# Dorothy-2016/rgbd360

Hardware: AMD Instinct MI355X
Metric: registered Frame360 pairs/sec @ 8×640×480; ICP-reduce HBM GB/s vs roofline (higher is better)
Workload: dtype f32

## Files before the change

### rgbd360_amd/csrc/kernels/plane_seg.hip

```cpp
#include <cstdio>
#include <cstdlib>
#include <cstring>
#include <type_traits>
#include "../r360_internal.h"
#include "../plane_math.h"

namespace {

__device__ __forceinline__ bool isfin(float v) { return __builtin_isfinite(v); }

__device__ __forceinline__ int ld(const int* p) { return __hip_atomic_load(p, __ATOMIC_RELAXED, __HIP_MEMORY_SCOPE_AGENT); }

__device__ int find_root(int* parent, int x) {
    int p = ld(parent + x);
    while (p != x) {
        const int gp = ld(parent + p);
        if (gp != p) __hip_atomic_store(parent + x, gp, __ATOMIC_RELAXED, __HIP_MEMORY_SCOPE_AGENT);
        x = gp;
        p = ld(parent + x);
    }
    return x;
}

__device__ void unite(int* parent, int a, int b) {
    while (true) {
        a = find_root(parent, a);
        b = find_root(parent, b);
        if (a == b) return;
        if (a < b) { const int t = a; a = b; b = t; }
        const int old = atomicCAS(parent + a, a, b);
        if (old == a) return;
        a = old;
    }
}

__device__ __forceinline__ bool plane_cmp(const float4& pa, const float4& na, const float4& nb, float ang_thr) {
    float thr = 0.02f;
    const float z = pa.x * 0.f + pa.y * 0.f + pa.z * 1.f;
    thr *= z * z;
    const float nd = na.x * nb.x + na.y * nb.y + na.z * nb.z;
    return fabsf(na.w - nb.w) < thr && nd > ang_thr;
}

constexpr int CCL_ROWS = 16, CCL_TPB = 1024;

__device__ int lds_find(int* lp, int x) {
    int p = lp[x];
    while (p != x) {
        const int gp = lp[p];
        if (gp != p) lp[x] = gp;
        x = gp;
        p = lp[x];
    }
    return x;
}

__device__ void lds_unite(int* lp, int a, int b) {
    while (true) {
        a = lds_find(lp, a);
        b = lds_find(lp, b);
        if (a == b) return;
        if (a < b) { const int t = a; a = b; b = t; }
        const int old = atomicCAS(lp + a, a, b);
        if (old == a) return;
        a = old;
    }
}

__device__ __forceinline__ void d_ccl_local(const float4* __restrict__ cloud, const float4* __restrict__ nrm,
                                                      int w, int h, float ang_thr, int* __restrict__ parent) {
    extern __shared__ int lp[];
    const int s = blockIdx.y, r0 = blockIdx.x * CCL_ROWS;
    if (r0 >= h) return;
    const int rows = min(CCL_ROWS, h - r0), n = rows * w;
    const long base = (long)s * w * h + (long)r0 * w;
    for (int k = threadIdx.x; k < n; k += CCL_TPB) lp[k] = isfin(cloud[base + k].x) ? k : -1;
    __syncthreads();
    for (int k = threadIdx.x; k < n; k += CCL_TPB) {
        if (lp[k] < 0) continue;
        const int rr = k / w, c = k - rr * w;
        const float4 p = cloud[base + k], nn = nrm[base + k];
        if (c >= 1 && lp[k - 1] >= 0 && plane_cmp(p, nn, nrm[base + k - 1], ang_thr)) lds_unite(lp, k, k - 1);
        if (rr >= 1 && lp[k - w] >= 0 && plane_cmp(p, nn, nrm[base + k - w], ang_thr)) lds_unite(lp, k, k - w);
    }
    __syncthreads();
    for (int k = threadIdx.x; k < n; k += CCL_TPB) {
        const int v = lp[k];
        parent[base + k] = v < 0 ? -1 : (int)(base + lds_find(lp, k));
    }
}
__global__ void __launch_bounds__(CCL_TPB) k_ccl_local(const PlaneBatch B, int w, int h, float ang_thr) {
    const PlaneDev& D = B.f[blockIdx.z];
    d_ccl_local(D.cloud, D.nrm, w, h, ang_thr, D.parent);
}


__device__ __forceinline__ void d_ccl_border(const float4* __restrict__ cloud, const float4* __restrict__ nrm, int w, int h,
                             float ang_thr, int* __restrict__ parent) {
    const int nb = (h - 1) / CCL_ROWS;
    const long total = 8L * nb * w;
    for (long t = blockIdx.x * (long)blockDim.x + threadIdx.x; t < total; t += (long)gridDim.x * blockDim.x) {
        const int s = (int)(t / ((long)nb * w));
        const int q = (int)(t - (long)s * nb * w);
        const int b = q / w, c = q - b * w;
        const long i = (long)s * w * h + (long)(b + 1) * CCL_ROWS * w + c;
        if (ld(parent + i) < 0 || ld(parent + i - w) < 0) continue;
        if (plane_cmp(cloud[i], nrm[i], nrm[i - w], ang_thr)) unite(parent, (int)i, (int)(i - w));
    }
}
__global__ void k_ccl_border(const PlaneBatch B, int w, int h, float ang_thr) {
    const PlaneDev& D = B.f[blockIdx.z];
    d_ccl_border(D.cloud, D.nrm, w, h, ang_thr, D.parent);
}


constexpr int NUMC = 256;

__device__ __forceinline__ void d_ccl_flatten(int* __restrict__ parent, int N, int* __restrict__ root,
                                                     int* __restrict__ cnt, int* __restrict__ ccnt) {
    const int s = blockIdx.y, j = blockIdx.x * NUMC + threadIdx.x;
    const long i = (long)s * N + j;
    bool is_root = false;
    if (j < N) {
        const int r = parent[i] < 0 ? -1 : find_root(parent, (int)i);
        root[i] = r;
        cnt[i] = 0;
        is_root = r == (int)i;
    }
    const int c = __syncthreads_count(is_root);
    if (threadIdx.x == 0) ccnt[s * gridDim.x + blockIdx.x] = c;
}
__global__ void __launch_bounds__(NUMC) k_ccl_flatten(const PlaneBatch B, int N) {
    const PlaneDev& D = B.f[blockIdx.z];
    d_ccl_flatten(D.parent, N, D.root, D.cnt, D.chunk);
}


__device__ __forceinline__ int chunk_rank(bool flag, const int* __restrict__ ccnt_s, int chunk, int& off, int& tot) {
    __shared__ int s_w[NUMC / 64], s_off[NUMC / 64];
    const int lane = threadIdx.x & 63, wid = threadIdx.x >> 6;
    int a = 0;
    for (int k = threadIdx.x; k < chunk; k += NUMC) a += ccnt_s[k];
    for (int o = 32; o > 0; o >>= 1) a += __shfl_xor(a, o, 64);
    const unsigned long long m = __ballot(flag);
    if (lane == 0) { s_off[wid] = a; s_w[wid] = __popcll(m); }
    __syncthreads();
    int o = 0, before = 0, t = 0;
    for (int w = 0; w < NUMC / 64; ++w) { o += s_off[w]; before += w < wid ? s_w[w] : 0; t += s_w[w]; }
    off = o;
    tot = t;
    return before + (int)__builtin_amdgcn_mbcnt_hi((unsigned)(m >> 32), __builtin_amdgcn_mbcnt_lo((unsigned)m, 0u));
}

__device__ __forceinline__ void d_ccl_number(const int* __restrict__ root, int N, const int* __restrict__ ccnt,
                                                    int* __restrict__ rank, int* __restrict__ nlab) {
    const int s = blockIdx.y, j = blockIdx.x * NUMC + threadIdx.x;
    const long i = (long)s * N + j;
    const bool is_root = j < N && root[i] == (int)i;
    int off, tot;
    const int r = chunk_rank(is_root, ccnt + s * gridDim.x, blockIdx.x, off, tot);
    if (is_root) rank[i] = off + r;
    if (blockIdx.x == gridDim.x - 1 && threadIdx.x == 0) nlab[s] = off + tot;
}
__global__ void __launch_bounds__(NUMC) k_ccl_number(const PlaneBatch B, int N) {
    const PlaneDev& D = B.f[blockIdx.z];
    d_ccl_number(D.root, N, D.chunk, D.parent, D.nlab);
}


__device__ __forceinline__ void d_ccl_label(const int* __restrict__ root, const int* __restrict__ rank, int N, int* __restrict__ lab,
                            int* __restrict__ cnt) {
    const long total = 8L * N;
    for (long i = blockIdx.x * (long)blockDim.x + threadIdx.x; i < total; i += (long)gridDim.x * blockDim.x) {
        const int rt = root[i];
        const int L = rt < 0 ? -1 : rank[rt];
        lab[i] = L;
        const int s = (int)(i / N);
        long key = L < 0 ? -1 : (long)s * N + L;
        bool pending = key >= 0;
        while (__any(pending)) {
            const unsigned long long act = __ballot(pending);
            const int leader = __ffsll((long long)act) - 1;
            const long lk = __shfl(key, leader, 64);
            const bool mine = pending && key == lk;
            const unsigned long long same = __ballot(mine);
            if (mine && (int)(threadIdx.x & 63) == leader) atomicAdd(cnt + lk, __popcll(same));
            if (mine) pending = false;
        }
    }
}
__global__ void k_ccl_label(const PlaneBatch B, int N) {
    const PlaneDev& D = B.f[blockIdx.z];
    d_ccl_label(D.root, D.parent, N, D.lab, D.cnt);
}


__device__ __forceinline__ void atomic_fmin(float* p, float v) {
    if (v >= 0.f) atomicMin(reinterpret_cast<int*>(p), __float_as_int(v));
    else atomicMax(reinterpret_cast<unsigned*>(p), __float_as_uint(v));
}
__device__ __forceinline__ void atomic_fmax(float* p, float v) {
    if (v >= 0.f) atomicMax(reinterpret_cast<int*>(p), __float_as_int(v));
    else atomicMin(reinterpret_cast<unsigned*>(p), __float_as_uint(v));
}

__device__ __forceinline__ void add128(unsigned long long* p, r360p::i128 v) {
    const unsigned long long lo = (unsigned long long)v, hi = (unsigned long long)(v >> 64);
    const unsigned long long old = atomicAdd(p, lo);
    atomicAdd(p + 1, hi + (old + lo < old ? 1ull : 0ull));
}

__device__ __forceinline__ void d_big_count(const int* __restrict__ cnt, const int* __restrict__ nlab, int N,
                                                   int min_inliers, int* __restrict__ bmap, int* __restrict__ ccnt) {
    const int s = blockIdx.y, j = blockIdx.x * NUMC + threadIdx.x;
    const long i = (long)s * N + j;
    bool big = false;
    if (j < nlab[s]) {
        big = cnt[i] > min_inliers;
        if (!big) bmap[i] = -1;
    }
    const int c = __syncthreads_count(big);
    if (threadIdx.x == 0) ccnt[s * gridDim.x + blockIdx.x] = c;
}
__global__ void __launch_bounds__(NUMC) k_big_count(const PlaneBatch B, int N, int min_inliers) {
    const PlaneDev& D = B.f[blockIdx.z];
    d_big_count(D.cnt, D.nlab, N, min_inliers, D.parent, D.chunk);
}


__device__ __forceinline__ void d_big_list(const int* __restrict__ cnt, const int* __restrict__ nlab, int N,
                                                  int min_inliers, const int* __restrict__ ccnt, int* __restrict__ big,
                                                  int* __restrict__ nbig, int maxbig, int* __restrict__ err,
                                                  int* __restrict__ bmap, r360p::Moments* __restrict__ mom,
                                                  int* __restrict__ bfirst) {
    const int s = blockIdx.y, j = blockIdx.x * NUMC + threadIdx.x;
    const long i = (long)s * N + j;
    const bool is_big = j < nlab[s] && cnt[i] > min_inliers;
    int off, tot;
    const int r = chunk_rank(is_big, ccnt + s * gridDim.x, blockIdx.x, off, tot);
    if (is_big) {
        const int b = off + r;
        bmap[i] = b < maxbig ? b : -1;
        if (b < maxbig) big[s * maxbig + b] = j;
    }
    if (blockIdx.x == gridDim.x - 1) {
        const int all = off + tot, nb = all < maxbig ? all : maxbig;
        if (threadIdx.x == 0) {
            nbig[s] = nb;
            if (all > maxbig) atomicOr(err, 2);
        }
        for (int q = threadIdx.x; q < nb; q += NUMC) {
            r360p::moments_zero(mom[s * maxbig + q]);
            bfirst[s * maxbig + q] = N;
        }
    }
}
__global__ void __launch_bounds__(NUMC) k_big_list(const PlaneBatch B, int N, int min_inliers, int maxbig) {
    const PlaneDev& D = B.f[blockIdx.z];
    d_big_list(D.cnt, D.nlab, N, min_inliers, D.chunk, D.big, D.nbig, maxbig, D.err, D.parent, D.mom, D.aux);
}


constexpr int GM_TPB = 256, GM_SLOTS = 64, GM_PX = 512, GM_COPIES = R360_GM_COPIES;


struct GmShared {
    int key[GM_SLOTS];
    unsigned long long w[GM_SLOTS][20];
    float b[GM_SLOTS][6];
    int first[GM_SLOTS];
};

struct GmAcc {
    long long n, s1[3], c[4];
    r360p::i128 s2[6];
    float b[6];
    int first;
};

__device__ __forceinline__ void gm_zero(GmAcc& a) {
    a.n = 0;
    a.first = 0x7fffffff;
    for (int k = 0; k < 3; ++k) a.s1[k] = 0;
    for (int k = 0; k < 4; ++k) a.c[k] = 0;
    for (int k = 0; k < 6; ++k) { a.s2[k] = 0; a.b[k] = k < 3 ? 3.4e38f : -3.4e38f; }
}


template <bool MODEL>
__device__ __forceinline__ void gm_deposit(GmShared* sh, int key, const GmAcc& a, r360p::Moments* gmom, int* gfirst,
                                           RegionPart* gout) {
    int h = key & (GM_SLOTS - 1), t = 0;
#pragma unroll 1
    for (; t < GM_SLOTS; ++t, h = (h + 1) & (GM_SLOTS - 1)) {
        const int old = atomicCAS(&sh->key[h], -1, key);
        if (old == -1 || old == key) break;
    }
    if (t < GM_SLOTS) {
        unsigned long long* d = sh->w[h];
        if (a.n) {
            atomicAdd(d + 0, (unsigned long long)a.n);
            for (int k = 0; k < 3; ++k) atomicAdd(d + 1 + k, (unsigned long long)a.s1[k]);
            for (int k = 0; k < 6; ++k) add128(d + 4 + 2 * k, a.s2[k]);
        }
        if (MODEL) {
            for (int k = 0; k < 4; ++k) atomicAdd(d + 16 + k, (unsigned long long)a.c[k]);
            for (int k = 0; k < 3; ++k) { atomic_fmin(&sh->b[h][k], a.b[k]); atomic_fmax(&sh->b[h][k + 3], a.b[k + 3]); }
        } else {
            atomicMin(&sh->first[h], a.first);
        }
        return;
    }
    r360p::Moments* dst = MODEL ? &gout[key].m : &gmom[key];
    if (a.n) {
        atomicAdd(reinterpret_cast<unsigned long long*>(&dst->n), (unsigned long long)a.n);
        for (int k = 0; k < 3; ++k) atomicAdd(reinterpret_cast<unsigned long long*>(&dst->s1[k]), (unsigned long long)a.s1[k]);
        for (int k = 0; k < 6; ++k) add128(reinterpret_cast<unsigned long long*>(&dst->s2[k]), a.s2[k]);
    }
    if (MODEL) {
        for (int k = 0; k < 4; ++k) atomicAdd(reinterpret_cast<unsigned long long*>(&dst->c[k]), (unsigned long long)a.c[k]);
        for (int k = 0; k < 3; ++k) { atomic_fmin(&gout[key].bmin[k], a.b[k]); atomic_fmax(&gout[key].bmax[k], a.b[k + 3]); }
    } else {
        atomicMin(gfirst + key, a.first);
    }
}

template <int CTRL>
__device__ __forceinline__ unsigned dpp32(unsigned v) {
    return (unsigned)__builtin_amdgcn_update_dpp(0, (int)v, CTRL, 0xf, 0xf, false);
}
template <int CTRL>
__device__ __forceinline__ long long dpp64(long long v) {
    const unsigned lo = dpp32<CTRL>((unsigned)(unsigned long long)v), hi = dpp32<CTRL>((unsigned)((unsigned long long)v >> 32));
    return (long long)(((unsigned long long)hi << 32) | lo);
}
template <int CTRL>
__device__ __forceinline__ r360p::i128 dpp128(r360p::i128 v) {
    const unsigned long long lo = (unsigned long long)dpp64<CTRL>((long long)(unsigned long long)v);
    const unsigned long long hi = (unsigned long long)dpp64<CTRL>((long long)(unsigned long long)(v >> 64));
    return (r360p::i128)(((unsigned __int128)hi << 64) | lo);
}
template <bool MODEL, int CTRL>
__device__ __forceinline__ void gm_scan_step(GmAcc& v, bool take) {
    long long s1[3];
    r360p::i128 s2[6];
    for (int k = 0; k < 3; ++k) s1[k] = dpp64<CTRL>(v.s1[k]);
    for (int k = 0; k < 6; ++k) s2[k] = dpp128<CTRL>(v.s2[k]);
    if (MODEL) {
        long long c[4];
        float b[6];
        for (int k = 0; k < 4; ++k) c[k] = dpp64<CTRL>(v.c[k]);
        for (int k = 0; k < 6; ++k) b[k] = __uint_as_float(dpp32<CTRL>(__float_as_uint(v.b[k])));
        if (take) {
            for (int k = 0; k < 4; ++k) v.c[k] += c[k];
            for (int k = 0; k < 3; ++k) { v.b[k] = fminf(v.b[k], b[k]); v.b[k + 3] = fmaxf(v.b[k + 3], b[k + 3]); }
        }
    }
    if (take) {
        for (int k = 0; k < 3; ++k) v.s1[k] += s1[k];
        for (int k = 0; k < 6; ++k) v.s2[k] += s2[k];
    }
}
template <bool MODEL>
__device__ __forceinline__ void gm_seg_scan(GmAcc& v, int lane, int head) {
    const int r = lane & 15, row = lane >> 4;
    gm_scan_step<MODEL, 0x111>(v, r >= 1 && head <= lane - 1);
    gm_scan_step<MODEL, 0x112>(v, r >= 2 && head <= lane - 2);
    gm_scan_step<MODEL, 0x114>(v, r >= 4 && head <= lane - 4);
    gm_scan_step<MODEL, 0x118>(v, r >= 8 && head <= lane - 8);
    gm_scan_step<MODEL, 0x142>(v, (row & 1) && head <= (lane & ~15) - 1);
    gm_scan_step<MODEL, 0x143>(v, row >= 2 && head <= 31);
}

template <bool MODEL, int CPW>
__device__ __forceinline__ void d_gm(const float4* __restrict__ cloud, const uchar4* __restrict__ rgb,
                                             const int* __restrict__ lab, int N, const int* __restrict__ kmap,
                                             int* __restrict__ mmap_clear, const float* __restrict__ rt8,
                                             r360p::Moments* __restrict__ gmom, int* __restrict__ gfirst,
                                             RegionPart* __restrict__ gpart, int exp) {
    __shared__ GmShared sh;
    RegionPart* const gout = MODEL ? gpart + (blockIdx.x % GM_COPIES) * 8 * R360_MAX_MODELS : nullptr;
    for (int q = threadIdx.x; q < GM_SLOTS; q += GM_TPB) {
        sh.key[q] = -1;
        sh.first[q] = 0x7fffffff;
        for (int k = 0; k < 20; ++k) sh.w[q][k] = 0;
        for (int k = 0; k < 6; ++k) sh.b[q][k] = k < 3 ? 3.4e38f : -3.4e38f;
    }
    const int lane = threadIdx.x & 63, wid = threadIdx.x >> 6;
    const long total = 8L * N;
    const long w0 = ((long)blockIdx.x * GM_TPB * CPW) + (long)wid * 64 * CPW + lane;
    int key[CPW];
#pragma unroll
    for (int c = 0; c < CPW; ++c) {
        const long i = w0 + 64 * c;
        key[c] = i < total ? lab[i] : -1;
        if (!MODEL && i < total) mmap_clear[i] = -1;
    }
#pragma unroll
    for (int c = 0; c < CPW; ++c) {
        const long i = w0 + 64 * c;
        const int s = (int)(i / N);
        const int m = key[c] >= 0 ? kmap[(long)s * N + key[c]] : -1;
        key[c] = m >= 0 ? s * (MODEL ? R360_MAX_MODELS : R360_MAX_BIG) + m : -1;
    }
    float4 pt[CPW];
    uchar4 col[CPW];
#pragma unroll
    for (int c = 0; c < CPW; ++c) {
        const long i = w0 + 64 * c;
        pt[c] = key[c] >= 0 ? cloud[i] : make_float4(0.f, 0.f, 0.f, 0.f);
        if (MODEL) col[c] = key[c] >= 0 ? rgb[i] : make_uchar4(0, 0, 0, 0);
    }
    __syncthreads();
#pragma unroll
    for (int c = 0; c < CPW; ++c) {
        const long i = w0 + 64 * c;
        const int s = (int)(i / N);
        GmAcc p;
        gm_zero(p);
        if (key[c] >= 0) {
            const float4 q = pt[c];
            float x = q.x, y = q.y, z = q.z;
            bool add = true;
            if (MODEL) {
                p.b[0] = q.x; p.b[1] = q.y; p.b[2] = q.z; p.b[3] = q.x; p.b[4] = q.y; p.b[5] = q.z;
                const float* T = rt8 + 16 * s;
                x = T[0] * q.x + T[4] * q.y + T[8] * q.z + T[12];
                y = T[1] * q.x + T[5] * q.y + T[9] * q.z + T[13];
                z = T[2] * q.x + T[6] * q.y + T[10] * q.z + T[14];
                const uchar4 cc = col[c];
                const int sum = cc.x + cc.y + cc.z;
                if (sum != 0) {
                    const float inv = 1.0f / float(sum);
                    p.c[0] = (long long)((double)(float(cc.x) * inv) * 8589934592.0);
                    p.c[1] = (long long)((double)(float(cc.y) * inv) * 8589934592.0);
                    p.c[2] = (long long)((double)(float(cc.z) * inv) * 8589934592.0);
                }
                p.c[3] = sum;
            } else {
                p.first = (int)(i - (long)s * N);
                add = isfin(q.x) && isfin(q.y) && isfin(q.z);
            }
            if (add) {
                const long long qv[3] = {r360p::q36(x), r360p::q36(y), r360p::q36(z)};
                p.n = 1;
                for (int k = 0; k < 3; ++k) p.s1[k] = qv[k];
                p.s2[0] = (r360p::i128)qv[0] * qv[0];
                p.s2[1] = (r360p::i128)qv[0] * qv[1];
                p.s2[2] = (r360p::i128)qv[0] * qv[2];
                p.s2[3] = (r360p::i128)qv[1] * qv[1];
                p.s2[4] = (r360p::i128)qv[1] * qv[2];
                p.s2[5] = (r360p::i128)qv[2] * qv[2];
            }
        }
        const unsigned long long heads = __ballot(lane == 0 || key[c] != __shfl_up(key[c], 1, 64));
        const unsigned long long le = lane == 63 ? ~0ull : (2ull << lane) - 1;
        const int head = 63 - __clzll((long long)(heads & le));
        const unsigned long long fin = __ballot(p.n != 0);
        if (!(exp & 4)) gm_seg_scan<MODEL>(p, lane, head);
        const bool tail = lane == 63 || ((heads >> (lane + 1)) & 1ull);
        if (!(exp & 2) && tail && key[c] >= 0) {
            const unsigned long long run = le & ~((1ull << head) - 1);
            p.n = __popcll(fin & run);
            p.first -= lane - head;
            gm_deposit<MODEL>(&sh, key[c], p, gmom, gfirst, gout);
        }
    }
    __syncthreads();
    for (int q = threadIdx.x >> 5; q < GM_SLOTS; q += GM_TPB / 32) {
        const int key = sh.key[q];
        if (key < 0 || (exp & 1)) continue;
        const int l = threadIdx.x & 31;
        r360p::Moments* dst = MODEL ? &gout[key].m : &gmom[key];
        if (l < 6) {
            unsigned long long* d = reinterpret_cast<unsigned long long*>(&dst->s2[l]);
            const unsigned long long lo = sh.w[q][4 + 2 * l], hi = sh.w[q][5 + 2 * l];
            const unsigned long long old = atomicAdd(d, lo);
            atomicAdd(d + 1, hi + (old + lo < old ? 1ull : 0ull));
        } else if (l < 14) {
            const int k = l - 6;
            if (k < 4 || MODEL) {
                long long* d = k == 0 ? &dst->n : k < 4 ? &dst->s1[k - 1] : &dst->c[k - 4];
                atomicAdd(reinterpret_cast<unsigned long long*>(d), sh.w[q][k == 0 ? 0 : k < 4 ? k : 12 + k]);
            }
        } else if (MODEL && l < 20) {
            const int k = l - 14;
            if (k < 3) atomic_fmin(&gout[key].bmin[k], sh.b[q][k]);
            else atomic_fmax(&gout[key].bmax[k - 3], sh.b[q][k]);
        } else if (!MODEL && l == 14) {
            atomicMin(gfirst + key, sh.first[q]);
        }
    }
}
template <bool MODEL, int CPW>
// ... 1426 lines not shown
        totals[1] = pre + x;
        if (pre + x > vox_cap) atomicOr(err, 16);
    }
}
__global__ void __launch_bounds__(512) k_vox_alloc(const PlaneBatch B) {
    const PlaneDev& D = B.f[blockIdx.z];
    d_vox_alloc(D.nmodels, D.out, D.totals, D.vox_cap, D.err);
}


constexpr int VOXC_TPB = 256;

template <typename F>
__device__ __forceinline__ void wave_by_key(int key, F&& f) {
    bool pending = key >= 0;
    while (__any(pending)) {
        const unsigned long long act = __ballot(pending);
        const int leader = __ffsll((long long)act) - 1;
        const int lk = __shfl(key, leader, 64);
        const bool mine = pending && key == lk;
        f(lk, __ballot(mine), leader, mine);
        if (mine) pending = false;
    }
}

__device__ __forceinline__ void d_vox_compact(VoxCell* __restrict__ tab,
                                                         const long* __restrict__ totals, PlaneOut* __restrict__ out,
                                                         VoxOut* __restrict__ pool, long pool_cap,
                                                         const int* __restrict__ vlist, const int* __restrict__ vcnt,
                                                         int px) {
    if (totals[3] == 0) return;
    const int n = vcnt[blockIdx.x];
    if (n == 0) return;
    __shared__ int cnt[8 * R360_MAX_MODELS], base[8 * R360_MAX_MODELS];
    for (int q = threadIdx.x; q < 8 * R360_MAX_MODELS; q += VOXC_TPB) cnt[q] = 0;
    __syncthreads();
    const int lane = threadIdx.x & 63;
    const int* L = vlist + (long)blockIdx.x * px;
    for (int kb = 0; kb < n; kb += VOXC_TPB) {
        const int k = kb + threadIdx.x;
        const unsigned long long tag = k < n ? tab[L[k]].tag : 0ull;
        wave_by_key(tag ? (int)(tag >> 48) - 1 : -1, [&](int key, unsigned long long m, int leader, bool) {
            if (lane == leader) atomicAdd(&cnt[key], __popcll(m));
        });
    }
    __syncthreads();
    for (int q = threadIdx.x; q < 8 * R360_MAX_MODELS; q += VOXC_TPB) {
        base[q] = cnt[q] ? atomicAdd(&out[q].vox_fill, cnt[q]) : 0;
        cnt[q] = 0;
    }
    __syncthreads();
    for (int kb = 0; kb < n; kb += VOXC_TPB) {
        const int k = kb + threadIdx.x;
        const int c = k < n ? L[k] : 0;
        const unsigned long long tag = k < n ? tab[c].tag : 0ull;
        const int sm = tag ? (int)(tag >> 48) - 1 : -1;
        int pos = 0;
        wave_by_key(sm, [&](int key, unsigned long long m, int leader, bool mine) {
            int o = 0;
            if (lane == leader) o = atomicAdd(&cnt[key], __popcll(m));
            o = __shfl(o, leader, 64);
            if (mine) pos = base[key] + o + (int)__builtin_amdgcn_mbcnt_hi((unsigned)(m >> 32),
                                                                            __builtin_amdgcn_mbcnt_lo((unsigned)m, 0u));
        });
        if (sm < 0) continue;
        const PlaneOut& O = out[sm];
        const double cn = (double)tab[c].cnt;
        VoxOut v;
        v.key = (long long)(tag & ((1ull << 48) - 1));
        v.x = (float)(tab[c].s[0] / cn);
        v.y = (float)(tab[c].s[1] / cn);
        v.z = (float)(tab[c].s[2] / cn);
        v.pad = 0.f;
        if (O.vox_off + pos < pool_cap) pool[O.vox_off + pos] = v;
        tab[c].tag = 0;
        tab[c].s[0] = tab[c].s[1] = tab[c].s[2] = 0.0;
        tab[c].cnt = 0;
    }
}
__global__ void __launch_bounds__(VOXC_TPB) k_vox_compact(const PlaneBatch B, int px) {
    const PlaneDev& D = B.f[blockIdx.z];
    d_vox_compact(D.vhash, D.totals, D.out, D.vox_dev, D.vox_cap, D.vlist, D.vcnt, px);
}

constexpr int VOXH_TPB = 256;
template <class PT>
__device__ __forceinline__ float pt_coord(const PT& v, int c) { return c == 0 ? v.x : c == 1 ? v.y : v.z; }

template <class PT>
__device__ __forceinline__ int d_hullpre(const PT* __restrict__ src, PT* __restrict__ dst, int n, const PlaneModel& model) {
    const int tid = threadIdx.x, lane = tid & 63, wid = tid >> 6;
    const float n0 = fabsf(model.v[0]), n1 = fabsf(model.v[1]), n2 = fabsf(model.v[2]);
    int k0 = n0 > n1 ? 0 : 1;
    k0 = (k0 == 0 ? n0 : n1) > n2 ? k0 : 2;
    const int ca = (k0 + 1) % 3, cb = (k0 + 2) % 3;
    __shared__ double s_v[VOXH_TPB];
    __shared__ int s_i[VOXH_TPB];
    __shared__ double s_best[8], s_ex[8], s_ey[8], s_vx[8], s_vy[8], s_M[8];
    __shared__ int s_idx[8], s_all, s_wc[VOXH_TPB / 64], s_base;
    double best[8];
    int bi[8];
    for (int k = 0; k < 8; ++k) { best[k] = -INFINITY; bi[k] = 0x7fffffff; }
    for (int i = tid; i < n; i += VOXH_TPB) {
        const double x = pt_coord(src[i], ca), y = pt_coord(src[i], cb);
        const double v[8] = {-x, -x - y, -y, x - y, x, x + y, y, y - x};
        for (int k = 0; k < 8; ++k)
            if (v[k] > best[k]) { best[k] = v[k]; bi[k] = i; }
    }
    for (int k = 0; k < 8; ++k) {
        s_v[tid] = best[k];
        s_i[tid] = bi[k];
        __syncthreads();
        for (int o = VOXH_TPB / 2; o > 0; o >>= 1) {
            if (tid < o) {
                const double a = s_v[tid], b = s_v[tid + o];
                const int ia = s_i[tid], ib = s_i[tid + o];
                if (b > a || (b == a && ib < ia)) { s_v[tid] = b; s_i[tid] = ib; }
            }
            __syncthreads();
        }
        if (tid == 0) { s_best[k] = s_v[0]; s_idx[k] = s_i[0]; }
        __syncthreads();
    }
    if (tid == 0) {
        double vx[8], vy[8];
        int mm = 0;
        for (int k = 0; k < 8; ++k) {
            const double x = pt_coord(src[s_idx[k]], ca), y = pt_coord(src[s_idx[k]], cb);
            if (mm && x == vx[mm - 1] && y == vy[mm - 1]) continue;
            vx[mm] = x; vy[mm] = y; ++mm;
        }
        if (mm > 1 && vx[mm - 1] == vx[0] && vy[mm - 1] == vy[0]) --mm;
        s_all = (n < 64 || mm < 3) ? 1 : 0;
        const double S = (s_best[4] + s_best[0]) + (s_best[6] + s_best[2]);
        for (int k = 0; k < 8; ++k) {
            const int e = k < mm ? k : 0, e1 = mm > 0 ? (e + 1) % mm : 0;
            s_ex[k] = mm > 0 ? vx[e1] - vx[e] : 0.0;
            s_ey[k] = mm > 0 ? vy[e1] - vy[e] : 0.0;
            s_vx[k] = mm > 0 ? vx[e] : 0.0;
            s_vy[k] = mm > 0 ? vy[e] : 0.0;
            s_M[k] = 1e-7 * (fabs(s_ex[k]) + fabs(s_ey[k])) * S;
        }
        s_base = 0;
    }
    __syncthreads();
    const bool all = s_all != 0;
    for (int i0 = 0; i0 < n; i0 += VOXH_TPB) {
        const int i = i0 + tid;
        bool keep = false;
        PT v;
        if (i < n) {
            v = src[i];
            keep = true;
            if (!all) {
                const double x = pt_coord(v, ca), y = pt_coord(v, cb);
                bool inside = true;
                for (int k = 0; k < 8; ++k) inside = inside && (s_ex[k] * (y - s_vy[k]) - s_ey[k] * (x - s_vx[k])) > s_M[k];
                keep = !inside;
            }
        }
        const unsigned long long bal = __ballot(keep);
        if (lane == 0) s_wc[wid] = __popcll(bal);
        __syncthreads();
        int off = s_base;
        for (int w = 0; w < wid; ++w) off += s_wc[w];
        if (keep) dst[off + (int)__builtin_amdgcn_mbcnt_hi((unsigned)(bal >> 32), __builtin_amdgcn_mbcnt_lo((unsigned)bal, 0u))] = v;
        __syncthreads();
        if (tid == 0) for (int w = 0; w < VOXH_TPB / 64; ++w) s_base += s_wc[w];
        __syncthreads();
    }
    return s_base;
}

__global__ void __launch_bounds__(VOXH_TPB) k_hullpre(const PlaneBatch B) {
    const PlaneDev& D = B.f[blockIdx.z];
    const int q = blockIdx.x, s = q / R360_MAX_MODELS, m = q % R360_MAX_MODELS;
    if (m >= D.nmodels[s]) return;
    PlaneOut& O = D.out[q];
    int kept = 0;
    if (O.n_contour > 0)
        kept = d_hullpre(D.contour_dev + O.contour_off, D.contour + O.contour_off, O.n_contour, O.model);
    else if (O.n_vox > 0 && D.totals[3] != 0)
        kept = d_hullpre(D.vox_dev + O.vox_off, D.vox + O.vox_off, O.n_vox, O.model);
    if (threadIdx.x == 0) O.hull_n = kept;
}
}


static unsigned long long g_force_fb_mask = 0;
static int g_force_fb_first = 0;

namespace {
__global__ void k_refine_force_fb(const PlaneBatch B, int w, int h, unsigned long long mask, int first_sweep) {
    const int f = blockIdx.x, s = blockIdx.y;
    if (!((mask >> (8 * f + s)) & 1ull)) return;
    const PlaneDev& D = B.f[f];
    int* fb = D.rflag;
    if (!first_sweep) {
        if (threadIdx.x == 0) fb[s] = (h - 1) / 2 + 1;
        return;
    }
    if (threadIdx.x == 0) { fb[s] = h - 1; fb[16 + s] = 1; }
    const long SK = (long)(h + w - 1) * h;
    for (long q = threadIdx.x; q < SK; q += blockDim.x) { D.rf1[s * SK + q] = -1; D.rf2[s * SK + q] = -1; }
}
}

extern "C" void r360_refine_force_fallback(uint64_t sensor_mask, int first_sweep) {
    g_force_fb_mask = sensor_mask;
    g_force_fb_first = first_sweep;
}

int refine_band_rows(int h) {
    static const int env = R360_KNOB("R360_REFINE_ROWS", -99);
    int rb = env >= -2 ? env : -1;
    if (rb < 0) return h <= 1024 ? rb : 0;
    if (rb > 0 && (h + rb - 1) / rb > R360_REFINE_BANDS) rb = (h + R360_REFINE_BANDS - 1) / R360_REFINE_BANDS;
    return rb;
}

int launch_refine_sweeps(const PlaneBatch& B, int F, hipStream_t st, int w, int h, int rb, bool wave_bufs, bool frame) {
    const int K = (w + 63) / 64;
    const unsigned nf = (unsigned)F;
    const int N = w * h;
    const dim3 px_grid((unsigned)((N + 255) / 256), 8, nf);
    const int blocks = (int)((8L * N + 255) / 256);
    if (rb < 0 && (w < 2 || h > 1024 || !wave_bufs)) rb = 0;
    if (rb < 0) {
        if (frame) hipLaunchKernelGGL(k_refine_prep<true>, px_grid, dim3(256), 0, st, B, w, h);
        else hipLaunchKernelGGL(k_refine_prep<false>, px_grid, dim3(256), 0, st, B, w, h);
        const int tpb = 64 * ((h + 63) / 64);
        const int narrow_max = 30;
        if (rb == -1 && h <= 64 * RP_MAXB && w <= RP_MAXW) {
            if (h <= 256) {
                hipLaunchKernelGGL((k_refine_pipe<1, 4>), dim3(8, 1, nf), dim3(tpb), 0, st, B, w, h, narrow_max);
                hipLaunchKernelGGL((k_refine_pipe<-1, 4>), dim3(8, 1, nf), dim3(tpb), 0, st, B, w, h, narrow_max);
            } else {
                hipLaunchKernelGGL((k_refine_pipe<1, RP_MAXB>), dim3(8, 1, nf), dim3(tpb), 0, st, B, w, h, narrow_max);
                hipLaunchKernelGGL((k_refine_pipe<-1, RP_MAXB>), dim3(8, 1, nf), dim3(tpb), 0, st, B, w, h, narrow_max);
            }
        } else {
            hipLaunchKernelGGL(k_refine_wave<1>, dim3(8, 1, nf), dim3(tpb), 0, st, B, w, h);
            hipLaunchKernelGGL(k_refine_wave<-1>, dim3(8, 1, nf), dim3(tpb), 0, st, B, w, h);
        }
        if (frame && g_force_fb_mask && h >= 2)
            hipLaunchKernelGGL(k_refine_force_fb, dim3(nf, 8), dim3(256), 0, st, B, w, h, g_force_fb_mask, g_force_fb_first);
        if (frame) hipLaunchKernelGGL(k_refine_finish, px_grid, dim3(256), 0, st, B, w, h);
        else hipLaunchKernelGGL(k_refine_unskew, dim3((unsigned)blocks, 1, nf), dim3(256), 0, st, B, w, h);
        switch (K) {
#define R360_FB_CASE(k)                                                                                         \
    case k:                                                                                                     \
        if (frame) hipLaunchKernelGGL((k_refine_fb<k, true>), dim3(8, 1, nf), dim3(64), 0, st, B, w, h);        \
        else hipLaunchKernelGGL((k_refine_fb<k, false>), dim3(8, 1, nf), dim3(64), 0, st, B, w, h);             \
        break;
            R360_FB_CASE(1) R360_FB_CASE(2) R360_FB_CASE(3) R360_FB_CASE(4) R360_FB_CASE(5)
            R360_FB_CASE(6) R360_FB_CASE(7) R360_FB_CASE(8) R360_FB_CASE(9) R360_FB_CASE(10)
#undef R360_FB_CASE
            default: r360_set_error("refine: cloud width %d > 640 unsupported", w); return -1;
        }
        R360_HIP(hipGetLastError());
        return 0;
    }
    if (rb > 0 && (h + rb - 1) / rb > R360_REFINE_BANDS) { r360_set_error("refine: %d rows per band too few", rb); return -2; }
    const int nb = rb > 0 ? (h + rb - 1) / rb : 0;
    if (frame) hipLaunchKernelGGL(k_refine_init, dim3(blocks, 1, nf), dim3(256), 0, st, B, N);
    switch (K) {
#define R360_REFINE_CASE(k)                                                                                     \
    case k:                                                                                                     \
        if (rb == 0) { hipLaunchKernelGGL(k_refine<k>, dim3(8, 1, nf), dim3(64), 0, st, B, w, h); break; }      \
        hipLaunchKernelGGL((k_refine_p1<k, 1>), dim3(nb, 8, nf), dim3(64), 0, st, B, w, h, rb);                 \
        hipLaunchKernelGGL((k_refine_p2<k, 1>), dim3(8, 1, nf), dim3(64), 0, st, B, w, h, rb, nb);              \
        hipLaunchKernelGGL((k_refine_p1<k, -1>), dim3(nb, 8, nf), dim3(64), 0, st, B, w, h, rb);                \
        hipLaunchKernelGGL((k_refine_p2<k, -1>), dim3(8, 1, nf), dim3(64), 0, st, B, w, h, rb, nb);             \
        break;
        R360_REFINE_CASE(1) R360_REFINE_CASE(2) R360_REFINE_CASE(3) R360_REFINE_CASE(4) R360_REFINE_CASE(5)
        R360_REFINE_CASE(6) R360_REFINE_CASE(7) R360_REFINE_CASE(8) R360_REFINE_CASE(9) R360_REFINE_CASE(10)
#undef R360_REFINE_CASE
        default: r360_set_error("refine: cloud width %d > 640 unsupported", w); return -1;
    }
    if (frame) hipLaunchKernelGGL(k_refine_final, dim3(blocks, 1, nf), dim3(256), 0, st, B, N);
    R360_HIP(hipGetLastError());
    return 0;
}

template <bool MODEL>
int launch_gm(int px, long total, const PlaneBatch& B, int F, hipStream_t st, int N) {
    const unsigned blocks = (unsigned)((total + px - 1) / px);
    const int exp = 0;
    switch (px) {
#define R360_GM_CASE(cpw)                                                                                         \
    case 256 * cpw:                                                                                               \
        hipLaunchKernelGGL((k_gm<MODEL, cpw>), dim3(blocks, 1, (unsigned)F), dim3(GM_TPB), 0, st, B, N, exp);    \
        return 0;
        R360_GM_CASE(1) R360_GM_CASE(2) R360_GM_CASE(4) R360_GM_CASE(8) R360_GM_CASE(16)
#undef R360_GM_CASE
    }
    r360_set_error("segmentation: R360_GM_PX=%d (256, 512, 1024, 2048 or 4096)", px);
    return -1;
}

int launch_segmentation_geom(const PlaneBatch& B, int F, const PlaneGeom& G, hipStream_t st, r360_ctx* tctx) {
    const int w = G.w, h = G.h, N = w * h;
    const long total = 8L * N;
    const int blocks = (int)((total + 255) / 256);
    const unsigned nf = (unsigned)F;
    const float ang_thr = cosf((float)0.039812);
    int slot = timing_begin(tctx, "k_ccl");
    hipLaunchKernelGGL(k_ccl_local, dim3((h + CCL_ROWS - 1) / CCL_ROWS, 8, nf), dim3(CCL_TPB), sizeof(int) * CCL_ROWS * w,
                       st, B, w, h, ang_thr);
    {
        const long edges = 8L * ((h - 1) / CCL_ROWS) * w;
        if (edges > 0)
            hipLaunchKernelGGL(k_ccl_border, dim3((unsigned)((edges + 255) / 256), 1, nf), dim3(256), 0, st, B, w, h, ang_thr);
    }
    const int nch = (N + NUMC - 1) / NUMC;
    hipLaunchKernelGGL(k_ccl_flatten, dim3(nch, 8, nf), dim3(NUMC), 0, st, B, N);
    hipLaunchKernelGGL(k_ccl_number, dim3(nch, 8, nf), dim3(NUMC), 0, st, B, N);
    hipLaunchKernelGGL(k_ccl_label, dim3(blocks, 1, nf), dim3(256), 0, st, B, N);
    timing_end(tctx, slot);
    R360_HIP(hipGetLastError());
    slot = timing_begin(tctx, "k_plane_fit");
    hipLaunchKernelGGL(k_big_count, dim3(nch, 8, nf), dim3(NUMC), 0, st, B, N, 80);
    hipLaunchKernelGGL(k_big_list, dim3(nch, 8, nf), dim3(NUMC), 0, st, B, N, 80, R360_MAX_BIG);
    static const int gm_px = R360_KNOB("R360_GM_PX", GM_PX);
    if (launch_gm<false>(gm_px, total, B, F, st, N)) return -1;
    hipLaunchKernelGGL(k_plane_fit, dim3(8, 1, nf), dim3(PF_TPB), 0, st, B, R360_MAX_BIG, 0.001f, N);
    timing_end(tctx, slot);
    R360_HIP(hipGetLastError());
    slot = timing_begin(tctx, "k_refine");
    if (launch_refine_sweeps(B, F, st, w, h, refine_band_rows(h), true, true)) return -1;
    timing_end(tctx, slot);
    R360_HIP(hipGetLastError());
    return 0;
}

int launch_segmentation_model(const PlaneBatch& B, int F, const PlaneGeom& G, hipStream_t st, r360_ctx* tctx) {
    const int w = G.w, h = G.h, N = w * h;
    const long total = 8L * N;
    const int blocks = (int)((total + 255) / 256);
    const unsigned nf = (unsigned)F;
    static const int gm_px = R360_KNOB("R360_GM_PX", GM_PX);
    int slot = timing_begin(tctx, "k_model_stats");
    if (launch_rgb(B, F, G, st)) return -1;
    if (launch_gm<true>(gm_px, total, B, F, st, N)) return -1;
    hipLaunchKernelGGL(k_nbmask, dim3(std::max(blocks, 20 * 8 * R360_MAX_MODELS / 256), 1, nf), dim3(256), 0, st, B, w, h);
    if (N <= TR_NB_MAX) hipLaunchKernelGGL(k_trace<true>, dim3(8, 1, nf), dim3(TR_TPB), 0, st, B, w, h);
    else hipLaunchKernelGGL(k_trace<false>, dim3(8, 1, nf), dim3(TR_TPB), 0, st, B, w, h);
    long cells, entries, groups;
    vox_scratch_need(G, &cells, &entries, &groups);
    const int vox_px = (int)(entries / groups);
    hipLaunchKernelGGL(k_alloc, dim3(1, 1, nf), dim3(512), 0, st, B);
    timing_end(tctx, slot);
    R360_HIP(hipGetLastError());
    slot = timing_begin(tctx, "k_voxel");
    hipLaunchKernelGGL(k_vox_hash, dim3((unsigned)groups, 1, nf), dim3(VOX_TPB), 0, st, B, N, vox_px);
    hipLaunchKernelGGL(k_vox_alloc, dim3(1, 1, nf), dim3(512), 0, st, B);
    hipLaunchKernelGGL(k_vox_compact, dim3((unsigned)groups, 1, nf), dim3(VOXC_TPB), 0, st, B, vox_px);
    hipLaunchKernelGGL(k_hullpre, dim3(8 * R360_MAX_MODELS, 1, nf), dim3(VOXH_TPB), 0, st, B);
    timing_end(tctx, slot);
    R360_HIP(hipGetLastError());
    return 0;
}

int launch_segmentation(const PlaneBatch& B, int F, const PlaneGeom& G, hipStream_t st, r360_ctx* tctx,
                        const hipEvent_t* bgr_ev) {
    if (launch_segmentation_geom(B, F, G, st, tctx)) return -1;
    for (int j = 0; bgr_ev && j < F; ++j)
        if (bgr_ev[j]) R360_HIP(hipStreamWaitEvent(st, bgr_ev[j], 0));
    return launch_segmentation_model(B, F, G, st, tctx);
}

void vox_scratch_need(const PlaneGeom& G, long* cells, long* entries, long* groups) {
    const int N = G.w * G.h;
    static const int vox_px_env = R360_KNOB("R360_VOX_PX", VOX_PX);
    const int vox_px = std::min(vox_px_env, N);
    const long vox_blocks = (8L * N + vox_px - 1) / vox_px;
    *cells = 12L * N;
    *entries = vox_blocks * vox_px;
    *groups = vox_blocks;
}

namespace {
__device__ __forceinline__ void d_plane_publish(const PlaneOut* __restrict__ out, const int* __restrict__ nmodels,
                                const int* __restrict__ err, const long* __restrict__ totals, PlaneOut* __restrict__ h_out,
                                int* __restrict__ h_nm, int nwords) {
    const int* src = reinterpret_cast<const int*>(out);
    int* dst = reinterpret_cast<int*>(h_out);
    constexpr int per = (int)(sizeof(PlaneOut) / 4);
    for (int i = blockIdx.x * blockDim.x + threadIdx.x; i < nwords; i += gridDim.x * blockDim.x) {
        const int slot = i / per;
        if (slot % R360_MAX_MODELS < nmodels[slot / R360_MAX_MODELS]) dst[i] = src[i];
    }
    if (blockIdx.x == 0 && threadIdx.x < 14 && threadIdx.x != 9) {
        const int t = threadIdx.x;
        h_nm[t] = t < 8 ? nmodels[t] : t == 8 ? *err : reinterpret_cast<const int*>(totals)[t - 10];
    }
}
__global__ void k_plane_publish(const PlaneBatch B, int nwords) {
    const PlaneDev& D = B.f[blockIdx.z];
    d_plane_publish(D.out, D.nmodels, D.err, D.totals, D.h_out, D.h_nmodels, nwords);
}

}

int launch_plane_publish(const PlaneBatch& B, int F, hipStream_t st) {
    static_assert(sizeof(PlaneOut) % 4 == 0, "PlaneOut is copied as 32-bit words");
    const int nwords = (int)(sizeof(PlaneOut) * 8 * R360_MAX_MODELS / 4);
    hipLaunchKernelGGL(k_plane_publish, dim3((nwords + 255) / 256, 1, (unsigned)F), dim3(256), 0, st, B, nwords);
    R360_HIP(hipGetLastError());
    return 0;
}

namespace {
__global__ void k_segment_inputs(const PlaneBatch B, long total) {
    const PlaneDev& D = B.f[blockIdx.z];
    if (blockIdx.x == 0 && threadIdx.x == 0) *D.err = 0;
    const float nan = __builtin_nanf("");
    for (long i = blockIdx.x * (long)blockDim.x + threadIdx.x; i < total; i += (long)gridDim.x * blockDim.x) {
        float4 p = D.cloud[i];
        p.w = 0.f;
        D.cloud[i] = p;
        const float4 n = D.nrm[i];
        float4 o = make_float4(nan, nan, nan, nan);
        if (isfin(n.x) && isfin(n.y) && isfin(n.z)) o = make_float4(n.x, n.y, n.z, p.x * n.x + p.y * n.y + p.z * n.z);
        D.nrm[i] = o;
    }
}
}

int launch_segment_inputs(const PlaneBatch& B, int F, const PlaneGeom& G, hipStream_t st) {
    const long total = 8L * G.w * G.h;
    const int blocks = (int)std::min<long>((total + 255) / 256, 4096);
    hipLaunchKernelGGL(k_segment_inputs, dim3(blocks, 1, (unsigned)F), dim3(256), 0, st, B, total);
    R360_HIP(hipGetLastError());
    return 0;
}

extern "C" int r360_refine_eval(const int8_t* state, const uint64_t* mask, int w, int h, int rb, int8_t* out) {
    if (!state || !mask || !out || w < 1 || h < 1 || w > 640) { r360_set_error("r360_refine_eval: bad arguments"); return -2; }
    const size_t T = 8 * (size_t)w * h;
    int8_t *S, *S2, *bnd;
    unsigned long long* MK;
    int* flag;
    R360_HIP(hipMalloc(&S, T));
    R360_HIP(hipMalloc(&S2, T));
    R360_HIP(hipMalloc(&MK, sizeof(unsigned long long) * T));
    R360_HIP(hipMalloc(&bnd, 8L * R360_REFINE_BANDS * w));
    R360_HIP(hipMalloc(&flag, sizeof(int) * 8 * R360_REFINE_BANDS));
    R360_HIP(hipMemcpy(S, state, T, hipMemcpyHostToDevice));
    R360_HIP(hipMemcpy(MK, mask, sizeof(unsigned long long) * T, hipMemcpyHostToDevice));
    uint16_t* code; unsigned long long* msk; int8_t *f1, *f2;
    const size_t SK = 8 * (size_t)(h + w - 1) * h;
    R360_HIP(hipMalloc(&code, sizeof(uint16_t) * SK));
    R360_HIP(hipMalloc(&msk, sizeof(unsigned long long) * SK));
    R360_HIP(hipMalloc(&f1, SK));
    R360_HIP(hipMalloc(&f2, SK));
    int nmh[8], *nm;
    for (int s = 0; s < 8; ++s) {
        int top = 0;
        for (size_t i = (size_t)s * w * h; i < (size_t)(s + 1) * w * h; ++i) {
            if (state[i] + 1 > top) top = state[i] + 1;
            if (mask[i]) top = std::max(top, 64 - __builtin_clzll(mask[i]));
        }
        nmh[s] = top;
    }
    R360_HIP(hipMalloc(&nm, sizeof(nmh)));
    R360_HIP(hipMemcpy(nm, nmh, sizeof(nmh), hipMemcpyHostToDevice));
    PlaneBatch B;
    std::memset(&B, 0, sizeof B);
    PlaneDev& D = B.f[0];
    D.state = S; D.state2 = S2; D.mask = MK; D.rbnd = bnd; D.rflag = flag;
    D.rcode = code; D.rmsk = msk; D.rf1 = f1; D.rf2 = f2; D.nmodels = nm;
    int rc = launch_refine_sweeps(B, 1, 0, w, h, rb, true, false);
    if (rc == 0) {
        R360_HIP(hipMemcpy(out, S, T, hipMemcpyDeviceToHost));
        if (rb < 0 && w >= 2 && h <= 1024) {
            int fbh[16];
            R360_HIP(hipMemcpy(fbh, flag, sizeof(fbh), hipMemcpyDeviceToHost));
            for (int k = 0; k < 8; ++k) rc += (fbh[k] != 0 || fbh[8 + k] != 0);
            if (R360_KNOB_STR("R360_REFINE_TRACE"))
                for (int k = 0; k < 8; ++k) fprintf(stderr, "refine sensor %d: re-runs %d fallback row %d\n", k, fbh[8 + k], fbh[k] - 1);
        }
    }
    (void)hipFree(S); (void)hipFree(S2); (void)hipFree(MK); (void)hipFree(bnd); (void)hipFree(flag); (void)hipFree(nm);
    (void)hipFree(code); (void)hipFree(msk); (void)hipFree(f1); (void)hipFree(f2);
    return rc;
}
```

Measured before the change: 2067.

## Aggregate CCL label counts in shared-memory hash table per block

Rewrites the label kernel so each block handles a contiguous chunk of one sensor. Adjacent equal labels within a wave are run-length merged, and counts are accumulated in a small open-addressed shared-memory hash table before being flushed to global memory. This replaces the per-wave leader election loop, which issued global atomics for every distinct label. It aims to cut global atomic traffic and contention, at the cost of shared-memory CAS probing and a fallback to global atomics when the table overflows.

```diff
diff --git a/rgbd360_amd/csrc/kernels/plane_seg.hip b/rgbd360_amd/csrc/kernels/plane_seg.hip
--- a/rgbd360_amd/csrc/kernels/plane_seg.hip
+++ b/rgbd360_amd/csrc/kernels/plane_seg.hip
@@ -168,28 +168,52 @@
 }
 
 
+constexpr int CL_TPB = 256, CL_CPW = 2, CL_PX = CL_TPB * CL_CPW, CL_SLOTS = 256, CL_PROBES = 8;
+
 __device__ __forceinline__ void d_ccl_label(const int* __restrict__ root, const int* __restrict__ rank, int N, int* __restrict__ lab,
                             int* __restrict__ cnt) {
-    const long total = 8L * N;
-    for (long i = blockIdx.x * (long)blockDim.x + threadIdx.x; i < total; i += (long)gridDim.x * blockDim.x) {
-        const int rt = root[i];
-        const int L = rt < 0 ? -1 : rank[rt];
-        lab[i] = L;
-        const int s = (int)(i / N);
-        long key = L < 0 ? -1 : (long)s * N + L;
-        bool pending = key >= 0;
-        while (__any(pending)) {
-            const unsigned long long act = __ballot(pending);
-            const int leader = __ffsll((long long)act) - 1;
-            const long lk = __shfl(key, leader, 64);
-            const bool mine = pending && key == lk;
-            const unsigned long long same = __ballot(mine);
-            if (mine && (int)(threadIdx.x & 63) == leader) atomicAdd(cnt + lk, __popcll(same));
-            if (mine) pending = false;
-        }
-    }
-}
-__global__ void k_ccl_label(const PlaneBatch B, int N) {
+    __shared__ int t_key[CL_SLOTS], t_cnt[CL_SLOTS];
+    for (int q = threadIdx.x; q < CL_SLOTS; q += CL_TPB) { t_key[q] = -1; t_cnt[q] = 0; }
+    const int lane = threadIdx.x & 63, wid = threadIdx.x >> 6;
+    const long base = (long)blockIdx.y * N;
+    const long j0 = (long)blockIdx.x * CL_PX + (long)wid * 64 * CL_CPW + lane;
+    int L[CL_CPW];
+#pragma unroll
+    for (int c = 0; c < CL_CPW; ++c) {
+        const long j = j0 + 64 * c;
+        L[c] = j < N ? root[base + j] : -1;
+    }
+#pragma unroll
+    for (int c = 0; c < CL_CPW; ++c) L[c] = L[c] < 0 ? -1 : rank[L[c]];
+#pragma unroll
+    for (int c = 0; c < CL_CPW; ++c) {
+        const long j = j0 + 64 * c;
+        if (j < N) lab[base + j] = L[c];
+    }
+    __syncthreads();
+#pragma unroll
+    for (int c = 0; c < CL_CPW; ++c) {
+        const int key = L[c];
+        const int prev = __shfl_up(key, 1, 64);
+        const unsigned long long heads = __ballot(lane == 0 || key != prev);
+        if (key >= 0 && ((heads >> lane) & 1ull)) {
+            const unsigned long long rest = lane == 63 ? 0ull : heads >> (lane + 1);
+            const int n = rest ? __ffsll((long long)rest) : 64 - lane;
+            int h = key & (CL_SLOTS - 1), t = 0;
+#pragma unroll 1
+            for (; t < CL_PROBES; ++t, h = (h + 1) & (CL_SLOTS - 1)) {
+                const int old = atomicCAS(&t_key[h], -1, key);
+                if (old == -1 || old == key) break;
+            }
+            if (t < CL_PROBES) atomicAdd(&t_cnt[h], n);
+            else atomicAdd(cnt + base + key, n);
+        }
+    }
+    __syncthreads();
+    for (int q = threadIdx.x; q < CL_SLOTS; q += CL_TPB)
+        if (t_key[q] >= 0) atomicAdd(cnt + base + t_key[q], t_cnt[q]);
+}
+__global__ void __launch_bounds__(CL_TPB) k_ccl_label(const PlaneBatch B, int N) {
     const PlaneDev& D = B.f[blockIdx.z];
     d_ccl_label(D.root, D.parent, N, D.lab, D.cnt);
 }
@@ -2222,7 +2246,6 @@
 int launch_segmentation_geom(const PlaneBatch& B, int F, const PlaneGeom& G, hipStream_t st, r360_ctx* tctx) {
     const int w = G.w, h = G.h, N = w * h;
     const long total = 8L * N;
-    const int blocks = (int)((total + 255) / 256);
     const unsigned nf = (unsigned)F;
     const float ang_thr = cosf((float)0.039812);
     int slot = timing_begin(tctx, "k_ccl");
@@ -2236,7 +2259,7 @@
     const int nch = (N + NUMC - 1) / NUMC;
     hipLaunchKernelGGL(k_ccl_flatten, dim3(nch, 8, nf), dim3(NUMC), 0, st, B, N);
     hipLaunchKernelGGL(k_ccl_number, dim3(nch, 8, nf), dim3(NUMC), 0, st, B, N);
-    hipLaunchKernelGGL(k_ccl_label, dim3(blocks, 1, nf), dim3(256), 0, st, B, N);
+    hipLaunchKernelGGL(k_ccl_label, dim3((N + CL_PX - 1) / CL_PX, 8, nf), dim3(CL_TPB), 0, st, B, N);
     timing_end(tctx, slot);
     R360_HIP(hipGetLastError());
     slot = timing_begin(tctx, "k_plane_fit");
```

Result: faster. 2096, median of 6 (+1.4%).
